# libjxl/libjxl

Measured on AMD Instinct MI355X. Metric: Mpixels/s decode (VarDCT d1.0, 8K RGB), higher is better.
Workload: dtype f32

## Files before the change

### libjxl_amd/csrc/entropy.cc

```cpp
#include "env_switches.h"
#include <stdlib.h>
namespace jxlhip_env {
Switches g;
void LoadLocked() {
  g.wp_general.store(getenv("JXLHIP_WP_GENERAL") != nullptr);
  g.codestream_verbose.store(getenv("JXLHIP_CODESTREAM_VERBOSE") != nullptr);
  g.no_pipeline.store(getenv("JXLHIP_NO_PIPELINE") != nullptr);
  const char* e = getenv("JXLHIP_TEST_RANGE_GROUP");
  g.test_range_group.store(e ? atoll(e) : -1);
  const char* ife = getenv("JXLHIP_MULTI_INTERIOR_FIRST");
  g.multi_interior_first.store(!ife || atoi(ife) != 0 ? 1 : 0);
  auto num = [](const char* name, int unset) {
    const char* v = getenv(name);
    return v ? atoi(v) : unset;
  };
  g.fused_pc_rh.store(num("JXLHIP_FUSED_PC_RH", 0));
  g.filter_rh.store(num("JXLHIP_FILTER_RH", 0));
  g.big_wgs.store(num("JXLHIP_BIG_WGS", Switches::kUnset));
  g.multi_force_gather.store(getenv("JXLHIP_MULTI_FORCE_GATHER") != nullptr);
  {
    const char* mp = getenv("JXLHIP_MAX_PIXELS");
    char* end = nullptr;
    const unsigned long long v = mp ? strtoull(mp, &end, 10) : 0ull;
    g.max_pixels.store((mp && end != mp && v != 0) ? v : (1ull << 30));
  }
  g.loaded.store(true, std::memory_order_release);
}
}
#include <math.h>
#include <stdlib.h>
#include <string.h>

#include <algorithm>
#include <functional>
#include <memory>
#include <mutex>
#include <new>
#include <vector>

#include "../../include/jxl_hip_entropy.h"
#include "../../include/jxl_hip_frame.h"

namespace {

constexpr int kOk = JXLHIP_OK;
constexpr int kBad = JXLHIP_ERR_BAD_STREAM;

class BitReader {
 public:
  BitReader(const uint8_t* data, size_t size, size_t bit_pos)
      : data_(data), size_(size), pos_(std::min(size, bit_pos / 8)) {
    if (bit_pos / 8 > size) overrun_ = true;
    Refill();
    Consume(bit_pos % 8);
  }
  inline void Refill() {
    if (size_ - pos_ >= 8 && pos_ <= size_) {
      uint64_t v;
      memcpy(&v, data_ + pos_, 8);
      buf_ |= v << nbits_;
      pos_ += (63 - nbits_) >> 3;
      nbits_ |= 56;
    } else {
      while (nbits_ <= 56) {
        const uint64_t b = pos_ < size_ ? data_[pos_] : 0;
        pos_++;
        buf_ |= b << nbits_;
        nbits_ += 8;
      }
    }
  }
  inline uint64_t Peek(uint32_t n) const { return buf_ & ((1ull << n) - 1ull); }
  inline void Consume(uint32_t n) {
    buf_ >>= n;
    nbits_ -= n;
  }
  inline uint32_t Read(uint32_t n) {
    Refill();
    const uint32_t v = (uint32_t)Peek(n);
    Consume(n);
    return v;
  }
  size_t BitsConsumed() const { return pos_ * 8 - nbits_; }
  bool Healthy() const { return !overrun_ && BitsConsumed() <= size_ * 8; }

 private:
  const uint8_t* data_;
  size_t size_;
  size_t pos_;
  uint64_t buf_ = 0;
  uint32_t nbits_ = 0;
  bool overrun_ = false;
};

inline uint32_t FloorLog2(uint32_t v) { return 31u - (uint32_t)__builtin_clz(v); }
inline uint32_t CeilLog2(uint32_t v) { return v <= 1 ? 0 : FloorLog2(v - 1) + 1; }

struct U32Dist {
  uint32_t bits[4];
  uint32_t offset[4];
};
uint32_t ReadU32(BitReader* br, const U32Dist& d) {
  const uint32_t sel = br->Read(2);
  return d.offset[sel] + (d.bits[sel] ? br->Read(d.bits[sel]) : 0);
}

constexpr int kRootBits = 8;
constexpr int kMaxCodeLength = 15;

struct PrefixEntry {
  uint8_t bits;
  uint16_t value;
};

struct PrefixCode {
  std::vector<PrefixEntry> table;

  inline uint32_t ReadSymbol(BitReader* br) const {
    const PrefixEntry* e = &table[br->Peek(kRootBits)];
    uint32_t n = e->bits;
    if (n > kRootBits) {
      br->Consume(kRootBits);
      e += e->value + br->Peek(n - kRootBits);
    }
    br->Consume(e->bits);
    return e->value;
  }

  void SetSingle(uint16_t symbol) {
    table.assign(1u << kRootBits, PrefixEntry{0, symbol});
  }

  bool Build(const uint8_t* lengths, size_t n, int root_bits) {
    uint32_t count[kMaxCodeLength + 1] = {0};
    for (size_t i = 0; i < n; i++) count[lengths[i]]++;
    uint32_t used = 0;
    for (int l = 1; l <= kMaxCodeLength; l++) used += count[l];
    const size_t root_size = (size_t)1 << root_bits;
    if (used == 0) return false;
    if (used == 1) {
      for (size_t i = 0; i < n; i++)
        if (lengths[i]) {
          table.assign(root_size, PrefixEntry{0, (uint16_t)i});
          return true;
        }
    }
    uint32_t space = 1u << kMaxCodeLength;
    for (int l = 1; l <= kMaxCodeLength; l++) {
      const uint32_t need = count[l] << (kMaxCodeLength - l);
      if (need > space) return false;
      space -= need;
    }
    if (space != 0) return false;
    uint32_t next_code[kMaxCodeLength + 2];
    {
      uint32_t code = 0;
      for (int l = 1; l <= kMaxCodeLength; l++) {
        next_code[l] = code;
        code = (code + count[l]) << 1;
      }
    }
    struct Sym {
      uint32_t rev;
      uint8_t len;
      uint16_t symbol;
    };
    std::vector<Sym> syms;
    syms.reserve(used);
    for (size_t i = 0; i < n; i++) {
      const int l = lengths[i];
      if (!l) continue;
// ... 2405 lines not shown
```

### libjxl_amd/csrc/env_switches.h

```cpp
#ifndef JXLHIP_ENV_SWITCHES_H_
#define JXLHIP_ENV_SWITCHES_H_
#include <atomic>
#include <mutex>

namespace jxlhip_env {
struct Switches {
  std::atomic<bool> loaded{false};
  std::atomic<bool> wp_general{false};
  std::atomic<bool> codestream_verbose{false};
  std::atomic<bool> no_pipeline{false};
  std::atomic<long long> test_range_group{-1};
  std::atomic<int> multi_interior_first{1};
  static constexpr int kUnset = -2147483647 - 1;
  std::atomic<int> fused_pc_rh{0};
  std::atomic<int> filter_rh{0};
  std::atomic<int> big_wgs{kUnset};
  std::atomic<bool> multi_force_gather{false};
  std::atomic<unsigned long long> max_pixels{1ull << 30};
  std::mutex mu;
};
extern Switches g;
void LoadLocked();
static inline const Switches& Get() {
  if (!g.loaded.load(std::memory_order_acquire)) {
    std::lock_guard<std::mutex> lock(g.mu);
    if (!g.loaded.load(std::memory_order_relaxed)) LoadLocked();
  }
  return g;
}
}
#endif
```

### libjxl_amd/csrc/kernels_blocks.hip

```cpp
#include <stdlib.h>
#include <string.h>

#include <type_traits>

#include <initializer_list>

#include "blocks_common.h"
#include "env_switches.h"

namespace jxlhip {

struct StrategyWord {
  uint32_t v[JXLHIP_NUM_STRATEGIES];
};
__host__ __device__ constexpr StrategyWord MakeStrategyWords() {
  StrategyWord w{};
  for (int s = 0; s < JXLHIP_NUM_STRATEGIES; s++)
    w.v[s] = (uint32_t)kCoveredX[s] | ((uint32_t)kCoveredY[s] << 8) | ((uint32_t)(uint8_t)ClassOfStrategy(s) << 16);
  return w;
}
__constant__ StrategyWord kStrategyWords = MakeStrategyWords();

__global__ __launch_bounds__(1024) void k_prepare(DevFrame f, WorkLists wl, uint32_t gy_lo,
                                                  int with_sigma, float epf_quant_mul,
// ... 403 lines not shown
  float v[64], px[64];
  {
    const uint4* p = (const uint4*)((const CT*)f.coeffs[1] + h.coef);
    uint4 raw[kVec];
#pragma unroll
    for (int i = 0; i < kVec; i++) raw[i] = p[i];
#pragma unroll
    for (int i = 0; i < kVec; i++) {
      int32_t q[kPer];
      unpack(raw[i], q);
#pragma unroll
      for (int k = 0; k < kPer; k++)
        v[i * kPer + k] = AdjustQuantBias(q[k], f.biases[1], f.biases[3]) * (tab[64 + i * kPer + k] * h.sy);
    }
  }
  if (c != 1) {
    const float sc = c == 0 ? h.sx : h.sb;
    const float cc = c == 0 ? h.x_cc : h.b_cc;
    const float bias = c == 0 ? f.biases[0] : f.biases[2];
    const float* __restrict__ tc = tab + c * 64;
    const uint4* p = (const uint4*)((const CT*)f.coeffs[c] + h.coef);
    uint4 raw[kVec];
#pragma unroll
    for (int i = 0; i < kVec; i++) raw[i] = p[i];
#pragma unroll
    for (int i = 0; i < kVec; i++) {
      int32_t q[kPer];
      unpack(raw[i], q);
#pragma unroll
      for (int k = 0; k < kPer; k++) {
        const float d = AdjustQuantBias(q[k], bias, f.biases[3]) * (tc[i * kPer + k] * sc);
        v[i * kPer + k] = __builtin_fmaf(cc, v[i * kPer + k], d);
      }
    }
  }
  v[0] = dcv;
  switch (strategy) {
    case 1: Transform64<1>(v, px); break;
    case 2: Transform64<2>(v, px); break;
    case 3: Transform64<3>(v, px); break;
    case 12: Transform64<12>(v, px); break;
    case 13: Transform64<13>(v, px); break;
    case 14: Transform64<14>(v, px); break;
    case 15: Transform64<15>(v, px); break;
    case 16: Transform64<16>(v, px); break;
    default: Transform64<17>(v, px); break;
  }
  if (valid) {
    float4* dst = (float4*)TilePtr(f, c, h.aby, h.abx);
#pragma unroll
    for (int i = 0; i < 16; i++) dst[i] = make_float4(px[4 * i], px[4 * i + 1], px[4 * i + 2], px[4 * i + 3]);
  }
}

template <typename CT>
__device__ __forceinline__ uint32_t SpecialWorkgroup(const DevFrame& f, const WorkLists& wl, uint32_t wg) {
  uint32_t cnt[kNumSpecial];
  uint32_t tasks = 0;
#pragma unroll
  for (int i = 0; i < kNumSpecial; i++) {
    cnt[i] = wl.count[(kClsSpecial0 + i) * kCounterPad];
    tasks += 3 * ((cnt[i] + 63) / 64);
  }
  const uint32_t special_wgs = (tasks + 3) / 4;
  if (wg >= special_wgs) return special_wgs;
  const uint32_t task = wg * 4 + (threadIdx.x >> 6);
  if (task >= tasks) return special_wgs;
  uint32_t base = 0;
  int cls = -1;
  uint32_t first = 0, n = 0, chan = 0;
#pragma unroll
  for (int i = 0; i < kNumSpecial; i++) {
    const uint32_t t = 3 * ((cnt[i] + 63) / 64);
    if (cls < 0 && task < base + t) {
      cls = i;
      first = ((task - base) / 3) * 64;
      chan = (task - base) % 3;
      n = cnt[i];
    }
    base += t;
  }
  SpecialTask<CT>(f, (int)kSpecialStrategy[cls], wl.list[kClsSpecial0 + cls], first, n,
                  chan == 0 ? 1 : (chan == 1 ? 0 : 2));
  return special_wgs;
}

template <typename CT>
__global__ __launch_bounds__(256, 3) void k_transform_8(DevFrame f, WorkLists wl) {
  const uint32_t special_wgs = SpecialWorkgroup<CT>(f, wl, blockIdx.x);
  if (blockIdx.x >= special_wgs)
    Dct8Rows<CT>(f, wl.list[kClsDct8], wl.count[kClsDct8 * kCounterPad], blockIdx.x - special_wgs);
}

template <int BIT>
__device__ __forceinline__ void ExchangePair(float& a, float& b, int lane) {
  if constexpr (BIT == 5) {
    SwapHalves32(a, b);
  } else if constexpr (BIT == 4) {
    SwapRows16(a, b);
  } else {
    const bool set = (lane >> BIT) & 1;
    const float send = set ? a : b;
    float recv;
    if constexpr (BIT == 3) {
      recv = __int_as_float(__builtin_amdgcn_update_dpp(0, __float_as_int(send), 0x128, 0xf, 0xf, false));
    } else if constexpr (BIT == 2) {
      const float lo = __int_as_float(__builtin_amdgcn_update_dpp(0, __float_as_int(send), 0x124, 0xf, 0xf, false));
      const float hi = __int_as_float(__builtin_amdgcn_update_dpp(0, __float_as_int(send), 0x12c, 0xf, 0xf, false));
      recv = set ? lo : hi;
    } else {
      static_assert(BIT == 1, "lane bits 1..5");
      recv = __int_as_float(__builtin_amdgcn_update_dpp(0, __float_as_int(send), 0x4e, 0xf, 0xf, false));
    }
    a = set ? recv : a;
    b = set ? b : recv;
  }
}

template <int S>
__device__ __forceinline__ void TransposeTile(float* w, int lane) {
  constexpr int kLog = S == 8 ? 3 : (S == 16 ? 4 : 5);
  constexpr int kLb0 = 6 - kLog;
#pragma unroll
  for (int t = kLog - 1; t >= 0; t--) {
#pragma unroll
    for (int k = 0; k < S; k++) {
      if (k & (1 << t)) continue;
      if (kLb0 + t == 5) ExchangePair<5>(w[k], w[k | (1 << t)], lane);
      else if (kLb0 + t == 4) ExchangePair<4>(w[k], w[k | (1 << t)], lane);
      else if (kLb0 + t == 3) ExchangePair<3>(w[k], w[k | (1 << t)], lane);
      else if (kLb0 + t == 2) ExchangePair<2>(w[k], w[k | (1 << t)], lane);
      else ExchangePair<1>(w[k], w[k | (1 << t)], lane);
    }
  }
}

typedef __attribute__((address_space(3))) float LdsTile;
template <int S>
__device__ __forceinline__ void TransposeTileLds(float* w, int b, int j, LdsTile* wave_lds) {
  LdsTile* tile = wave_lds + b * (S * (S + 1));
  LdsTile* row = tile + j * (S + 1);
#pragma unroll
  for (int a = 0; a < S; a++) row[a] = w[a];
  __builtin_amdgcn_fence(__ATOMIC_RELEASE, "wavefront");
  __builtin_amdgcn_wave_barrier();
  __builtin_amdgcn_fence(__ATOMIC_ACQUIRE, "wavefront");
#pragma unroll
  for (int a = 0; a < S; a++) w[a] = tile[a * (S + 1) + j];
  __builtin_amdgcn_fence(__ATOMIC_RELEASE, "wavefront");
  __builtin_amdgcn_wave_barrier();
}
template <int S>
constexpr int TransposeLdsBytes() { return 4 * (64 / S) * S * (S + 1) * 4; }

template <int R, int C, int STRATEGY, typename CT, bool LDS_T = false>
__device__ __forceinline__ void RowLaneUnit(const DevFrame& f, const WorkItem* __restrict__ list,
                                            uint32_t first, uint32_t n, unsigned char* smem = nullptr) {
  constexpr int S = R < C ? R : C, L = R < C ? C : R;
  constexpr int BPS = 64 / S;
  constexpr int CY = R / 8, CX = C / 8;
  constexpr int kTiles = L / S;
  constexpr int kVec = L * (int)sizeof(CT) / 16;
  const int tid = Tid();
  const int lane = tid & 63, wave = tid >> 6;
  const int j = lane / BPS;
  const uint32_t vb = first + wave * BPS + (lane & (BPS - 1));
  if (first + wave * BPS >= n) return;
  const bool valid = vb < n;
  const WorkItem it = list[valid ? vb : n - 1];
  const BlockHdr h = MakeHdr(f, it);
  uint4 raw_a[kVec], raw_b[kVec];
  auto request = [&](int c, uint4* r) {
    const uint4* p = (const uint4*)((const CT*)f.coeffs[c] + h.coef + (size_t)j * L);
#pragma unroll
    for (int i = 0; i < kVec; i++) r[i] = p[i];
  };
  request(1, raw_a);
  request(0, raw_b);
  constexpr int kLlfLanes = CY < CX ? CY : CX;
  constexpr int kLlfRegs = CY < CX ? CX : CY;
  auto llf_of = [&](int c, float* out) {
    const float* dc = f.dc[c] + (size_t)h.aby * f.xsb + h.abx;
    float dp[CY][CX];
#pragma unroll
    for (int x = 0; x < CX; x++) {
      float v[CY];
#pragma unroll
      for (int y = 0; y < CY; y++) v[y] = dc[(size_t)y * f.xsb + x];
      DctReg<CY>(v);
#pragma unroll
      for (int y = 0; y < CY; y++) dp[y][x] = (1.0f / CY) * v[y];
    }
#pragma unroll
    for (int y = 0; y < CY; y++) {
      float v[CX];
#pragma unroll
      for (int x = 0; x < CX; x++) v[x] = dp[y][x];
      DctReg<CX>(v);
      const float ry = kResampleUpHost[CY + y];
#pragma unroll
      for (int x = 0; x < CX; x++) {
        const float val = (1.0f / CX) * v[x];
        if constexpr (CY < CX) {
          if (j == y) out[x] = val * ry * kResampleUpHost[CX + x];
        } else {
          if (j == x) out[y] = val * kResampleUpHost[CX + x] * ry;
        }
      }
    }
  };
  const float* __restrict__ tab = f.dequant + DequantOffset(STRATEGY) + j * L;
  constexpr int kPer = 16 / (int)sizeof(CT);
  auto unpack_piece = [&](const uint4 r, int32_t* q) {
    if constexpr (sizeof(CT) == 2) {
      const uint32_t w[4] = {r.x, r.y, r.z, r.w};
#pragma unroll
      for (int k = 0; k < 4; k++) {
        q[2 * k] = (int32_t)(int16_t)(w[k] & 0xffffu);
        q[2 * k + 1] = (int32_t)w[k] >> 16;
      }
    } else {
      q[0] = (int32_t)r.x, q[1] = (int32_t)r.y, q[2] = (int32_t)r.z, q[3] = (int32_t)r.w;
    }
  };
  float vy[L];
#pragma unroll
  for (int i = 0; i < kVec; i++) {
    int32_t q[kPer];
    unpack_piece(raw_a[i], q);
#pragma unroll
    for (int k = 0; k < kPer; k++)
      vy[i * kPer + k] = AdjustQuantBias(q[k], f.biases[1], f.biases[3]) * (tab[R * C + i * kPer + k] * h.sy);
    if constexpr (L > 16) __builtin_amdgcn_sched_barrier(0);
  }
  request(2, raw_a);
#pragma unroll
  for (int ci = 0; ci < 3; ci++) {
    const int c = ci == 0 ? 1 : (ci == 1 ? 0 : 2);
    float v[L];
    if (c == 1) {
#pragma unroll
      for (int k = 0; k < L; k++) v[k] = vy[k];
    } else {
      const float sc = c == 0 ? h.sx : h.sb;
      const float cc = c == 0 ? h.x_cc : h.b_cc;
#pragma unroll
      for (int i = 0; i < kVec; i++) {
        int32_t q[kPer];
        unpack_piece(c == 0 ? raw_b[i] : raw_a[i], q);
#pragma unroll
        for (int k = 0; k < kPer; k++) {
          const float d = AdjustQuantBias(q[k], f.biases[c], f.biases[3]) * (tab[c * R * C + i * kPer + k] * sc);
          v[i * kPer + k] = __builtin_fmaf(cc, vy[i * kPer + k], d);
        }
        if constexpr (L > 16) __builtin_amdgcn_sched_barrier(0);
      }
    }
    if (j < kLlfLanes) {
      float llf[kLlfRegs];
      llf_of(c, llf);
#pragma unroll
      for (int k = 0; k < kLlfRegs; k++) v[k] = llf[k];
    }
    IdctReg<L>(v);
#pragma unroll
    for (int t = 0; t < kTiles; t++) {
      if constexpr (LDS_T) TransposeTileLds<S>(v + t * S, lane & (BPS - 1), j, (LdsTile*)smem + wave * (BPS * S * (S + 1)));
      else TransposeTile<S>(v + t * S, lane);
    }
#pragma unroll
    for (int t = 0; t < kTiles; t++) IdctReg<S>(v + t * S);
    if constexpr (R < C) {
#pragma unroll
      for (int t = 0; t < kTiles; t++) {
        if constexpr (LDS_T) TransposeTileLds<S>(v + t * S, lane & (BPS - 1), j, (LdsTile*)smem + wave * (BPS * S * (S + 1)));
        else TransposeTile<S>(v + t * S, lane);
      }
      if (valid) {
#pragma unroll
        for (int g = 0; g < C / 8; g++) {
          float* dst = TilePtr(f, c, h.aby + (j >> 3), h.abx + g) + (j & 7) * 8;
          *(float4*)dst = make_float4(v[g * 8], v[g * 8 + 1], v[g * 8 + 2], v[g * 8 + 3]);
          *(float4*)(dst + 4) = make_float4(v[g * 8 + 4], v[g * 8 + 5], v[g * 8 + 6], v[g * 8 + 7]);
        }
      }
    } else {
      if (valid) {
#pragma unroll
        for (int t = 0; t < kTiles; t++) {
          const int a = t * S + j;
#pragma unroll
          for (int g = 0; g < C / 8; g++) {
            float* dst = TilePtr(f, c, h.aby + (a >> 3), h.abx + g) + (a & 7) * 8;
            const float* src = v + t * S + g * 8;
            *(float4*)dst = make_float4(src[0], src[1], src[2], src[3]);
            *(float4*)(dst + 4) = make_float4(src[4], src[5], src[6], src[7]);
          }
        }
      }
    }
  }
}

template <int N>
__device__ __forceinline__ float ResampleUpSel(int i) {
  float r = kResampleUpHost[N];
#pragma unroll
  for (int j = 1; j < N; j++) r = (i == j) ? kResampleUpHost[N + j] : r;
  return r;
}

template <int R, int C>
struct MediumGeom {
  static constexpr int S = R < C ? R : C, L = R < C ? C : R;
  static constexpr int ML = L;
  static constexpr int NB = 64 / ML;
  static constexpr int LP = L + 1;
  static constexpr int TP = C + 1;
  static constexpr int BUF = (S * LP > R * TP ? S * LP : R * TP);
  static constexpr int CY = R / 8, CX = C / 8;
  static constexpr int kUnitVarblocks = (64 / (CY * CX)) > NB ? 64 / (CY * CX) : NB;
  static constexpr int kHdrOffset = (12 * NB * (BUF + CY * CX) + 15) & ~15;
  static constexpr bool kPipelined = (NB * R * C + 767) / 768 <= 2;
  static constexpr int kTabOffset = kHdrOffset + kUnitVarblocks * 48;
  static constexpr int kLdsBytes = kTabOffset + (kPipelined ? 12 * R * C : 0);
};

template <int R, int C, typename CT>
struct MediumLoads {
  using G = MediumGeom<R, C>;
  static constexpr int SIZE = R * C;
  static constexpr int kSteps = (G::NB * SIZE + 767) / 768;
  static constexpr bool kPipelined = G::kPipelined;
  using Raw = typename std::conditional<sizeof(CT) == 2, uint2, int4>::type;
  Raw x[kSteps], y[kSteps], b[kSteps];
  float dc[G::CY];
};

template <typename CT>
__device__ __forceinline__ void UnpackCoeffs(const uint2 v, int32_t* q) {
  q[0] = (int16_t)(v.x & 0xffff);
  q[1] = (int32_t)v.x >> 16;
  q[2] = (int16_t)(v.y & 0xffff);
  q[3] = (int32_t)v.y >> 16;
}
template <typename CT>
__device__ __forceinline__ void UnpackCoeffs(const int4 v, int32_t* q) {
  q[0] = v.x;
  q[1] = v.y;
  q[2] = v.z;
  q[3] = v.w;
}

template <int R, int C, typename CT>
__device__ __forceinline__ void MediumFetch(const DevFrame& f, const BlockHdr* hdr, int nb,
                                            MediumLoads<R, C, CT>& ld) {
  using G = MediumGeom<R, C>;
  using LD = MediumLoads<R, C, CT>;
  using Raw = typename LD::Raw;
  const int tid = Tid();
  const int c = tid >> 6, lane = tid & 63;
  const int b = lane / G::ML, i = lane % G::ML;
  if (b < nb && i < G::CX) {
    const BlockHdr& h = hdr[b];
    const float* dc = f.dc[c] + (size_t)h.aby * f.xsb + h.abx + i;
#pragma unroll
    for (int y = 0; y < G::CY; y++) ld.dc[y] = dc[(size_t)y * f.xsb];
  }
#pragma unroll
  for (int it = 0; it < LD::kSteps; it++) {
    const int k4 = tid * 4 + it * 768;
    if (k4 < nb * LD::SIZE) {
      const int vb = k4 / LD::SIZE, k = k4 % LD::SIZE;
      const size_t at = hdr[vb].coef + k;
      ld.x[it] = *(const Raw*)((const CT*)f.coeffs[0] + at);
      ld.y[it] = *(const Raw*)((const CT*)f.coeffs[1] + at);
      ld.b[it] = *(const Raw*)((const CT*)f.coeffs[2] + at);
    }
  }
}

struct TabStep {
  float4 x, y, b;
};

template <int R, int C, int STRATEGY, typename CT>
__device__ __forceinline__ void MediumBatch(const DevFrame& f, const BlockHdr* hdr, int nb,
                                            const MediumLoads<R, C, CT>& ld, unsigned char* smem) {
  using G = MediumGeom<R, C>;
  using LD = MediumLoads<R, C, CT>;
  constexpr int L = G::L, ML = G::ML, NB = G::NB, LP = G::LP, TP = G::TP, BUF = G::BUF;
  constexpr int CY = G::CY, CX = G::CX;
  constexpr int SIZE = R * C;
  constexpr uint32_t kTab = DequantOffset(STRATEGY);
  float(*buf)[NB][BUF] = reinterpret_cast<float(*)[NB][BUF]>(smem);
  float(*dcp)[NB][CY * CX] = reinterpret_cast<float(*)[NB][CY * CX]>(smem + 12 * NB * BUF);
  const int tid = Tid();

  const int c = tid >> 6, lane = tid & 63;
  const int b = lane / ML, i = lane % ML;
  const bool active = b < nb;
  const int bb = active ? b : 0;
  float* m = &buf[c][bb][0];
  float* dp = &dcp[c][bb][0];

// ... 480 lines not shown
struct UnitPick {
  int index;
  int cls;
  uint32_t first;
  uint32_t n;
};

template <int N>
__device__ __forceinline__ UnitPick PickUnit(const FamilyEntry (&fam)[N], const uint32_t* cnt,
                                             uint32_t u) {
  UnitPick p{-1, 0, 0, 0};
  uint32_t base = 0;
#pragma unroll
  for (int i = 0; i < N; i++) {
    const uint32_t units = (cnt[i] + fam[i].unit_varblocks - 1) / fam[i].unit_varblocks;
    if (p.index < 0 && u < base + units) {
      p.index = i;
      p.cls = fam[i].cls;
      p.first = (u - base) * fam[i].unit_varblocks;
      p.n = cnt[i];
    }
    base += units;
  }
  return p;
}

static constexpr int kLdsFamilyA = MediumGeom<64, 64>::kLdsBytes;
static_assert(TransposeLdsBytes<32>() <= kLdsFamilyA && TransposeLdsBytes<16>() <= kLdsFamilyA && TransposeLdsBytes<8>() <= kLdsFamilyA,
              "the row-per-lane units of k_transform_r transpose through family A's allocation");
static_assert(sizeof(BlockHdr) <= 48, "header slots are 48 bytes");
static_assert(MediumGeom<64, 32>::kLdsBytes <= kLdsFamilyA && MediumGeom<32, 64>::kLdsBytes <= kLdsFamilyA, "");

static constexpr FamilyEntry kFamilyA[3] = {{kClsMedium0 + 8, 1}, {kClsMedium0 + 9, 2}, {kClsMedium0 + 10, 2}};
static constexpr FamilyEntry kFamilyR16[3] = {{kClsMedium0 + 2, 16}, {kClsMedium0 + 0, 32}, {kClsMedium0 + 1, 32}};
static constexpr FamilyEntry kFamilyR32[5] = {{kClsMedium0 + 7, 8},  {kClsMedium0 + 5, 16}, {kClsMedium0 + 6, 16},
                                              {kClsMedium0 + 3, 32}, {kClsMedium0 + 4, 32}};
static_assert(kMediumStrategy[8] == 18 && kMediumStrategy[9] == 19 && kMediumStrategy[10] == 20 &&
              kMediumStrategy[7] == 5 && kMediumStrategy[5] == 10 && kMediumStrategy[6] == 11 &&
              kMediumStrategy[2] == 4 && kMediumStrategy[3] == 8 && kMediumStrategy[4] == 9 &&
              kMediumStrategy[0] == 6 && kMediumStrategy[1] == 7, "class table mismatch");

template <int N, typename Body>
__device__ __forceinline__ void UnitDispatch(const FamilyEntry (&fam)[N], const WorkLists& wl,
                                             Body&& body, uint32_t wg_index, uint32_t num_wgs,
                                             uint32_t skip_mask = 0) {
  uint32_t cnt[N];
#pragma unroll
  for (int i = 0; i < N; i++)
    cnt[i] = (skip_mask >> i) & 1u ? 0u : wl.count[fam[i].cls * kCounterPad];
  for (uint32_t u = wg_index;; u += num_wgs) {
    const UnitPick pick = PickUnit(fam, cnt, u);
    if (pick.index < 0) return;
    body(pick.index, wl.list[pick.cls], pick.first, pick.n);
    __syncthreads();
  }
}

static constexpr FamilyEntry kFamilyA1[3] = {{kClsMedium0 + 8, 1}, {kClsMedium0 + 9, 1}, {kClsMedium0 + 10, 1}};

__device__ __forceinline__ void FamilyALoop16(const DevFrame& f, const WorkLists& wl, unsigned char* smem, uint32_t wg_index,
                                              uint32_t num_wgs) {
  uint32_t cnt[3];
#pragma unroll
  for (int i = 0; i < 3; i++) cnt[i] = wl.count[kFamilyA1[i].cls * kCounterPad];
  uint32_t u = wg_index;
  UnitPick cur = PickUnit(kFamilyA1, cnt, u);
  if (cur.index < 0) return;
  BlockHdr hc = MakeHdr(f, wl.list[cur.cls][cur.first]);
  APrefetch P;
#define JXLHIP_AREQUEST(INDEX, H)                      \
  switch (INDEX) {                                     \
    case 0: ARequest<64, 64, 18>(f, H, P); break;      \
    case 1: ARequest<64, 32, 19>(f, H, P); break;      \
    default: ARequest<32, 64, 20>(f, H, P); break;     \
  }
  JXLHIP_AREQUEST(cur.index, hc)
  for (;;) {
    const UnitPick nxt = PickUnit(kFamilyA1, cnt, u + num_wgs);
    WorkItem in{};
    if (nxt.index >= 0) in = wl.list[nxt.cls][nxt.first];
    switch (cur.index) {
      case 0: AHead<64, 64, 18>(f, hc, P, smem); break;
      case 1: AHead<64, 32, 19>(f, hc, P, smem); break;
      default: AHead<32, 64, 20>(f, hc, P, smem); break;
    }
    BlockHdr hn{};
    if (nxt.index >= 0) {
      hn = MakeHdr(f, in);
      JXLHIP_AREQUEST(nxt.index, hn)
    }
    switch (cur.index) {
      case 0: AStore<64, 64>(f, hc, smem); break;
      case 1: AStore<64, 32>(f, hc, smem); break;
      default: AStore<32, 64>(f, hc, smem); break;
    }
    if (nxt.index < 0) return;
    __syncthreads();
    cur = nxt;
    hc = hn;
    u += num_wgs;
  }
#undef JXLHIP_AREQUEST
}

template <typename CT>
__global__ __launch_bounds__(192, sizeof(CT) == 2 ? 3 : 2) void k_transform_a(DevFrame f, WorkLists wl) {
  __shared__ __attribute__((aligned(16))) unsigned char smem[kLdsFamilyA];
  if constexpr (sizeof(CT) == 2) {
    FamilyALoop16(f, wl, smem, blockIdx.x, gridDim.x);
  } else {
    UnitDispatch(kFamilyA, wl,
                 [&](int index, const WorkItem* __restrict__ list, uint32_t first, uint32_t n) {
                   switch (index) {
                     case 0: MediumUnit<64, 64, 18, CT>(f, list, first, n, smem); break;
                     case 1: MediumUnit<64, 32, 19, CT>(f, list, first, n, smem); break;
                     default: MediumUnit<32, 64, 20, CT>(f, list, first, n, smem); break;
                   }
                 },
                 blockIdx.x, gridDim.x);
  }
}

template <typename CT>
__global__ __launch_bounds__(256) void k_transform_r16(DevFrame f, WorkLists wl) {
  UnitDispatch(kFamilyR16, wl,
               [&](int index, const WorkItem* __restrict__ list, uint32_t first, uint32_t n) {
                 switch (index) {
                   case 0: RowLaneUnit<16, 16, 4, CT>(f, list, first, n); break;
                   case 1: RowLaneUnit<16, 8, 6, CT>(f, list, first, n); break;
                   default: RowLaneUnit<8, 16, 7, CT>(f, list, first, n); break;
                 }
               },
               blockIdx.x, gridDim.x, f.mfma16 != nullptr ? 1u : 0u);
}

template <typename CT>
__global__ __launch_bounds__(256) void k_transform_r32(DevFrame f, WorkLists wl) {
  UnitDispatch(kFamilyR32, wl,
               [&](int index, const WorkItem* __restrict__ list, uint32_t first, uint32_t n) {
                 switch (index) {
                   case 0: RowLaneUnit<32, 32, 5, CT>(f, list, first, n); break;
                   case 1: RowLaneUnit<32, 16, 10, CT>(f, list, first, n); break;
                   case 2: RowLaneUnit<16, 32, 11, CT>(f, list, first, n); break;
                   case 3: RowLaneUnit<32, 8, 8, CT>(f, list, first, n); break;
                   default: RowLaneUnit<8, 32, 9, CT>(f, list, first, n); break;
                 }
               },
               blockIdx.x, gridDim.x, f.mfma32 != nullptr ? 1u : 0u);
}

static constexpr FamilyEntry kFamilyR[8] = {{kClsMedium0 + 7, 8},  {kClsMedium0 + 5, 16}, {kClsMedium0 + 6, 16},
                                            {kClsMedium0 + 3, 32}, {kClsMedium0 + 4, 32}, {kClsMedium0 + 2, 16},
                                            {kClsMedium0 + 0, 32}, {kClsMedium0 + 1, 32}};
template <typename CT>
__global__ __launch_bounds__(256, sizeof(CT) == 2 ? 3 : 2) void k_transform_r(DevFrame f, WorkLists wl, uint32_t big_wgs,
                                                                               uint32_t special_wgs, uint32_t r_wgs,
                                                                               uint32_t dct8_wgs) {
  __shared__ __attribute__((aligned(16))) unsigned char smem[kLdsFamilyA];
  if (blockIdx.x < special_wgs) {
    SpecialWorkgroup<CT>(f, wl, blockIdx.x);
    return;
  }
  const uint32_t np = big_wgs + r_wgs;
  const uint32_t i = blockIdx.x - special_wgs;
  const uint32_t need8 = (wl.count[kClsDct8 * kCounterPad] + Dct8Geom<CT>::kPerWg - 1) / Dct8Geom<CT>::kPerWg;
  const uint32_t d8 = need8 * 4 < dct8_wgs ? need8 : dct8_wgs;
  const uint32_t pairs = np < d8 ? np : d8;
  bool is_dct8;
  uint32_t idx;
  if (i < 2 * pairs) {
    is_dct8 = (i & 1u) != 0;
    idx = i >> 1;
  } else {
    is_dct8 = d8 > np;
    idx = i - pairs;
    if (idx >= (is_dct8 ? d8 : np)) return;
  }
  if (is_dct8) {
    Dct8Rows<CT>(f, wl.list[kClsDct8], wl.count[kClsDct8 * kCounterPad], idx);
    return;
  }
  if (idx < big_wgs) {
    if (threadIdx.x >= 192) return;
    if constexpr (sizeof(CT) == 2) {
      FamilyALoop16(f, wl, smem, idx, big_wgs);
    } else {
      UnitDispatch(kFamilyA, wl,
                   [&](int index, const WorkItem* __restrict__ list, uint32_t first, uint32_t n) {
                     switch (index) {
                       case 0: MediumUnit<64, 64, 18, CT>(f, list, first, n, smem); break;
                       case 1: MediumUnit<64, 32, 19, CT>(f, list, first, n, smem); break;
                       default: MediumUnit<32, 64, 20, CT>(f, list, first, n, smem); break;
                     }
                   },
                   idx, big_wgs);
    }
    return;
  }
  UnitDispatch(kFamilyR, wl,
               [&](int index, const WorkItem* __restrict__ list, uint32_t first, uint32_t n) {
                 switch (index) {
                   case 0: RowLaneUnit<32, 32, 5, CT, true>(f, list, first, n, smem); break;
                   case 1: RowLaneUnit<32, 16, 10, CT, true>(f, list, first, n, smem); break;
                   case 2: RowLaneUnit<16, 32, 11, CT, true>(f, list, first, n, smem); break;
                   case 3: RowLaneUnit<32, 8, 8, CT, true>(f, list, first, n, smem); break;
                   case 4: RowLaneUnit<8, 32, 9, CT, true>(f, list, first, n, smem); break;
                   case 5: RowLaneUnit<16, 16, 4, CT, true>(f, list, first, n, smem); break;
                   case 6: RowLaneUnit<16, 8, 6, CT, true>(f, list, first, n, smem); break;
                   default: RowLaneUnit<8, 16, 7, CT, true>(f, list, first, n, smem); break;
                 }
               },
               idx - big_wgs, r_wgs, (f.mfma32 != nullptr ? 1u : 0u) | (f.mfma16 != nullptr ? 1u << 5 : 0u));
}

template <typename CT>
static void LaunchBlocksT(const DevFrame& f, const WorkLists& wl, uint32_t cells, const float* wc,
                          const float* resample, hipStream_t* streams, int nstreams, const FilterParams* emit) {
  const uint32_t units = cells / 64;
  const uint32_t grid_l = cells / 128 < 512u ? (cells / 128 ? cells / 128 : 1) : 512u;
  constexpr uint32_t kDct8PerWg = Dct8Geom<CT>::kPerWg;
  const uint32_t grid_a = units + 3 < 1536u ? units + 3 : 1536u;
  const uint32_t grid_r16 = units + 3 < 4096u ? units + 3 : 4096u;
  const uint32_t grid_r32 = units / 2 + 5 < 3072u ? units / 2 + 5 : 3072u;
  hipStream_t s0 = streams[0], s1 = streams[1 % nstreams];
  auto any = [&](std::initializer_list<int> strategies) {
    if (f.used_acs == 0) return true;
    for (int st : strategies)
      if (f.used_acs & (1u << st)) return true;
    return false;
  };
  const bool need_r16 = any({6, 7}) || (!f.mfma16 && any({4}));
  const bool need_r32 = any({8, 9, 10, 11}) || (!f.mfma32 && any({5}));
  const bool merged_r = need_r16 && need_r32;
  const bool have_big = any({18, 19, 20});
  bool specials_in_r = false, dct8_in_r = false;
  uint32_t grid_specials = 0, grid_dct8 = 0;
  if (have_big && !merged_r)
    hipLaunchKernelGGL((k_transform_a<CT>), dim3(grid_a), dim3(192), 0, s1, f, wl);
  {
    const bool specials = any({1, 2, 3, 12, 13, 14, 15, 16, 17});
    const uint32_t bound_s = specials ? (cells / 64 + kNumSpecial) * 3 / 4 + 1 : 0;
    const uint32_t cells_8 = f.fused == 0 ? cells : (f.fused == 2 ? 2u * f.xsb : 0u);
    const uint32_t bound_8 = (any({0}) && cells_8) ? (cells_8 + kDct8PerWg - 1) / kDct8PerWg : 0;
    const uint32_t grid_8 = (bound_s > bound_8 ? bound_s : bound_8) + (specials ? kNumSpecial : 0);
    specials_in_r = merged_r && specials;
    dct8_in_r = merged_r && bound_8 != 0;
    grid_specials = bound_s + kNumSpecial;
    grid_dct8 = bound_8;
    if (grid_8 && !merged_r) hipLaunchKernelGGL((k_transform_8<CT>), dim3(grid_8), dim3(256), 0, s0, f, wl);
  }
  if (merged_r) {
    uint32_t big_cap = 512u;
    const int big_env = jxlhip_env::Get().big_wgs.load(std::memory_order_relaxed);
    if (big_env >= 1 && big_env <= 4096) big_cap = (uint32_t)big_env;
    const uint32_t big_wgs = have_big ? (grid_a < big_cap ? grid_a : big_cap) : 0u;
    const uint32_t special_wgs = specials_in_r ? grid_specials : 0u;
    const uint32_t dct8_wgs = dct8_in_r ? grid_dct8 : 0u;
    hipLaunchKernelGGL((k_transform_r<CT>), dim3(special_wgs + big_wgs + grid_r16 + dct8_wgs), dim3(256), 0, s0, f, wl,
                       big_wgs, special_wgs, grid_r16, dct8_wgs);
  } else {
    if (need_r16) hipLaunchKernelGGL((k_transform_r16<CT>), dim3(grid_r16), dim3(256), 0, s0, f, wl);
    if (need_r32) hipLaunchKernelGGL((k_transform_r32<CT>), dim3(grid_r32), dim3(256), 0, s0, f, wl);
  }
  if (f.mfma32 && any({5})) LaunchMfma32(f, wl, cells, s1, emit);
  if (f.mfma16 && any({4})) LaunchMfma16(f, wl, cells, s1);
  if (cells >= 256 && any({21, 22, 23, 24, 25, 26}))
    hipLaunchKernelGGL(k_large<CT>, dim3(grid_l), dim3(256), 0, s1, f, wl.list[kClsLarge],
                       wl.count + kClsLarge * kCounterPad, wc, resample);
}

void LaunchPrepare(const DevFrame& f, const WorkLists& wl, int with_sigma, float epf_quant_mul,
                   const SharpLut& lut, hipStream_t st) {
  uint32_t lo = f.band_g0, hi = f.band_g1;
  if (with_sigma) {
    if (lo == f.group_y0 && lo > 0) lo--;
    if (hi == f.group_y0 + f.group_rows && hi < f.ysg) hi++;
  }
  hipLaunchKernelGGL(k_prepare, dim3(f.xsg * (hi - lo)), dim3(1024), 0, st, f, wl, lo,
                     with_sigma, epf_quant_mul, lut);
}

void LaunchBlocks(const DevFrame& f, const WorkLists& wl, uint32_t cells, const float* wc,
                  const float* resample, hipStream_t* streams, int nstreams, const FilterParams* emit) {
  if (f.coeff_type == JXLHIP_COEFF_I16)
    LaunchBlocksT<int16_t>(f, wl, cells, wc, resample, streams, nstreams, emit);
  else
    LaunchBlocksT<int32_t>(f, wl, cells, wc, resample, streams, nstreams, emit);
}

}
```

Before: 113,100.

## Stage dequant tables and DC patches in LDS for row-per-lane units

After: 116,000, median of 6. +2.6%, better.

```diff
diff --git a/libjxl_amd/csrc/entropy.cc b/libjxl_amd/csrc/entropy.cc
--- a/libjxl_amd/csrc/entropy.cc
+++ b/libjxl_amd/csrc/entropy.cc
@@ -17,6 +17,7 @@
   g.fused_pc_rh.store(num("JXLHIP_FUSED_PC_RH", 0));
   g.filter_rh.store(num("JXLHIP_FILTER_RH", 0));
   g.big_wgs.store(num("JXLHIP_BIG_WGS", Switches::kUnset));
+  g.r_wgs.store(num("JXLHIP_R_WGS", Switches::kUnset));
   g.multi_force_gather.store(getenv("JXLHIP_MULTI_FORCE_GATHER") != nullptr);
   {
     const char* mp = getenv("JXLHIP_MAX_PIXELS");
diff --git a/libjxl_amd/csrc/env_switches.h b/libjxl_amd/csrc/env_switches.h
--- a/libjxl_amd/csrc/env_switches.h
+++ b/libjxl_amd/csrc/env_switches.h
@@ -15,6 +15,7 @@
   std::atomic<int> fused_pc_rh{0};
   std::atomic<int> filter_rh{0};
   std::atomic<int> big_wgs{kUnset};
+  std::atomic<int> r_wgs{kUnset};
   std::atomic<bool> multi_force_gather{false};
   std::atomic<unsigned long long> max_pixels{1ull << 30};
   std::mutex mu;
diff --git a/libjxl_amd/csrc/kernels_blocks.hip b/libjxl_amd/csrc/kernels_blocks.hip
--- a/libjxl_amd/csrc/kernels_blocks.hip
+++ b/libjxl_amd/csrc/kernels_blocks.hip
@@ -579,6 +579,10 @@
 }
 template <int S>
 constexpr int TransposeLdsBytes() { return 4 * (64 / S) * S * (S + 1) * 4; }
+static constexpr int kRlTabOff = TransposeLdsBytes<32>();
+static constexpr int kRlDcOff = kRlTabOff + 3 * 32 * 32 * 4;
+static constexpr int kRlDcWaveFloats = 96;
+static constexpr int kRlLdsBytes = kRlDcOff + 4 * kRlDcWaveFloats * 4;
 
 template <int R, int C, int STRATEGY, typename CT, bool LDS_T = false>
 __device__ __forceinline__ void RowLaneUnit(const DevFrame& f, const WorkItem* __restrict__ list,
@@ -596,6 +600,21 @@
   const bool valid = vb < n;
   const WorkItem it = list[valid ? vb : n - 1];
   const BlockHdr h = MakeHdr(f, it);
+  constexpr int kDcN = (R / 8) * (C / 8);
+  static_assert(BPS * 3 * kDcN <= kRlDcWaveFloats && 3 * kDcN <= 2 * S, "DC staging geometry");
+  LdsTile* dcl = (LdsTile*)(smem + kRlDcOff) + wave * kRlDcWaveFloats + (lane & (BPS - 1)) * (3 * kDcN);
+  float dcs[2] = {0.0f, 0.0f};
+  if constexpr (LDS_T) {
+#pragma unroll
+    for (int r = 0; r < 2; r++) {
+      const int e = j + r * S;
+      if (e < 3 * kDcN) {
+        const int c = e / kDcN, y = (e % kDcN) / (C / 8), x = e % (C / 8);
+        const float* dcp = c == 0 ? f.dc[0] : (c == 1 ? f.dc[1] : f.dc[2]);
+        dcs[r] = dcp[(size_t)(h.aby + y) * f.xsb + h.abx + x];
+      }
+    }
+  }
   uint4 raw_a[kVec], raw_b[kVec];
   auto request = [&](int c, uint4* r) {
     const uint4* p = (const uint4*)((const CT*)f.coeffs[c] + h.coef + (size_t)j * L);
@@ -604,6 +623,11 @@
   };
   request(1, raw_a);
   request(0, raw_b);
+  if constexpr (LDS_T) {
+#pragma unroll
+    for (int r = 0; r < 2; r++)
+      if (j + r * S < 3 * kDcN) dcl[j + r * S] = dcs[r];
+  }
   constexpr int kLlfLanes = CY < CX ? CY : CX;
   constexpr int kLlfRegs = CY < CX ? CX : CY;
   auto llf_of = [&](int c, float* out) {
@@ -613,7 +637,10 @@
     for (int x = 0; x < CX; x++) {
       float v[CY];
 #pragma unroll
-      for (int y = 0; y < CY; y++) v[y] = dc[(size_t)y * f.xsb + x];
+      for (int y = 0; y < CY; y++) {
+        if constexpr (LDS_T) v[y] = dcl[c * kDcN + y * CX + x];
+        else v[y] = dc[(size_t)y * f.xsb + x];
+      }
       DctReg<CY>(v);
 #pragma unroll
       for (int y = 0; y < CY; y++) dp[y][x] = (1.0f / CY) * v[y];
@@ -636,7 +663,12 @@
       }
     }
   };
-  const float* __restrict__ tab = f.dequant + DequantOffset(STRATEGY) + j * L;
+  const float* __restrict__ tab_g = f.dequant + DequantOffset(STRATEGY) + j * L;
+  const LdsTile* tab_l = (const LdsTile*)(smem + kRlTabOff) + j * L;
+  auto tab = [&](int i) -> float {
+    if constexpr (LDS_T) return tab_l[i];
+    else return tab_g[i];
+  };
   constexpr int kPer = 16 / (int)sizeof(CT);
   auto unpack_piece = [&](const uint4 r, int32_t* q) {
     if constexpr (sizeof(CT) == 2) {
@@ -657,7 +689,7 @@
     unpack_piece(raw_a[i], q);
 #pragma unroll
     for (int k = 0; k < kPer; k++)
-      vy[i * kPer + k] = AdjustQuantBias(q[k], f.biases[1], f.biases[3]) * (tab[R * C + i * kPer + k] * h.sy);
+      vy[i * kPer + k] = AdjustQuantBias(q[k], f.biases[1], f.biases[3]) * (tab(R * C + i * kPer + k) * h.sy);
     if constexpr (L > 16) __builtin_amdgcn_sched_barrier(0);
   }
   request(2, raw_a);
@@ -677,7 +709,7 @@
         unpack_piece(c == 0 ? raw_b[i] : raw_a[i], q);
 #pragma unroll
         for (int k = 0; k < kPer; k++) {
-          const float d = AdjustQuantBias(q[k], f.biases[c], f.biases[3]) * (tab[c * R * C + i * kPer + k] * sc);
+          const float d = AdjustQuantBias(q[k], f.biases[c], f.biases[3]) * (tab(c * R * C + i * kPer + k) * sc);
           v[i * kPer + k] = __builtin_fmaf(cc, vy[i * kPer + k], d);
         }
         if constexpr (L > 16) __builtin_amdgcn_sched_barrier(0);
@@ -1464,6 +1496,15 @@
 static constexpr FamilyEntry kFamilyR[8] = {{kClsMedium0 + 7, 8},  {kClsMedium0 + 5, 16}, {kClsMedium0 + 6, 16},
                                             {kClsMedium0 + 3, 32}, {kClsMedium0 + 4, 32}, {kClsMedium0 + 2, 16},
                                             {kClsMedium0 + 0, 32}, {kClsMedium0 + 1, 32}};
+template <int R, int C, int STRATEGY>
+__device__ __forceinline__ void RowLaneTables(const DevFrame& f, unsigned char* smem) {
+  static_assert(DequantOffset(STRATEGY) % 4 == 0, "16-byte table pieces");
+  const float4* src = (const float4*)(f.dequant + DequantOffset(STRATEGY));
+  float4* dst = (float4*)(smem + kRlTabOff);
+  for (int i = (int)threadIdx.x; i < 3 * R * C / 4; i += 256) dst[i] = src[i];
+}
+static_assert(kRlLdsBytes <= kLdsFamilyA, "the row-per-lane units' tables and DC patches fit family A's allocation");
+
 template <typename CT>
 __global__ __launch_bounds__(256, sizeof(CT) == 2 ? 3 : 2) void k_transform_r(DevFrame f, WorkLists wl, uint32_t big_wgs,
                                                                                uint32_t special_wgs, uint32_t r_wgs,
@@ -1509,8 +1550,23 @@
     }
     return;
   }
+  int tab_index = -1;
   UnitDispatch(kFamilyR, wl,
                [&](int index, const WorkItem* __restrict__ list, uint32_t first, uint32_t n) {
+                 if (index != tab_index) {
+                   switch (index) {
+                     case 0: RowLaneTables<32, 32, 5>(f, smem); break;
+                     case 1: RowLaneTables<32, 16, 10>(f, smem); break;
+                     case 2: RowLaneTables<16, 32, 11>(f, smem); break;
+                     case 3: RowLaneTables<32, 8, 8>(f, smem); break;
+                     case 4: RowLaneTables<8, 32, 9>(f, smem); break;
+                     case 5: RowLaneTables<16, 16, 4>(f, smem); break;
+                     case 6: RowLaneTables<16, 8, 6>(f, smem); break;
+                     default: RowLaneTables<8, 16, 7>(f, smem); break;
+                   }
+                   __syncthreads();
+                   tab_index = index;
+                 }
                  switch (index) {
                    case 0: RowLaneUnit<32, 32, 5, CT, true>(f, list, first, n, smem); break;
                    case 1: RowLaneUnit<32, 16, 10, CT, true>(f, list, first, n, smem); break;
@@ -1566,10 +1622,12 @@
     const int big_env = jxlhip_env::Get().big_wgs.load(std::memory_order_relaxed);
     if (big_env >= 1 && big_env <= 4096) big_cap = (uint32_t)big_env;
     const uint32_t big_wgs = have_big ? (grid_a < big_cap ? grid_a : big_cap) : 0u;
+    const int r_env = jxlhip_env::Get().r_wgs.load(std::memory_order_relaxed);
+    const uint32_t r_wgs = r_env >= 1 && r_env <= 4096 ? (uint32_t)r_env : grid_r16;
     const uint32_t special_wgs = specials_in_r ? grid_specials : 0u;
     const uint32_t dct8_wgs = dct8_in_r ? grid_dct8 : 0u;
-    hipLaunchKernelGGL((k_transform_r<CT>), dim3(special_wgs + big_wgs + grid_r16 + dct8_wgs), dim3(256), 0, s0, f, wl,
-                       big_wgs, special_wgs, grid_r16, dct8_wgs);
+    hipLaunchKernelGGL((k_transform_r<CT>), dim3(special_wgs + big_wgs + r_wgs + dct8_wgs), dim3(256), 0, s0, f, wl,
+                       big_wgs, special_wgs, r_wgs, dct8_wgs);
   } else {
     if (need_r16) hipLaunchKernelGGL((k_transform_r16<CT>), dim3(grid_r16), dim3(256), 0, s0, f, wl);
     if (need_r32) hipLaunchKernelGGL((k_transform_r32<CT>), dim3(grid_r32), dim3(256), 0, s0, f, wl);
```
